# PrimeIntellect-ai/prime

Hardware: AMD Instinct MI355X
Metric: tokens_per_sec (higher is better)
Workload: dtype bf16; 1 GPU; model=intellect_10b, global_batch=8, seq_len=2048, parallelism=diloco1_h100_int8ring

## Files before the change

prime_amd/ops/_lib.py:

```python
from __future__ import annotations

import ctypes
from typing import Optional

import torch

from .build import LIB_PATH, build, needs_build

_LIB: Optional[ctypes.CDLL] = None
_TRIED = False

_SIGS = {
    "prime_rmsnorm_fwd": [ctypes.c_void_p] * 5 + [ctypes.c_int64] * 2 + [ctypes.c_double],
    "prime_rmsnorm_bwd": [ctypes.c_void_p] * 7 + [ctypes.c_int64] * 3 + [ctypes.c_double],
    "prime_add_rmsnorm_fwd": [ctypes.c_void_p] * 7 + [ctypes.c_int64] * 2 + [ctypes.c_double],
    "prime_add_rmsnorm_bwd": [ctypes.c_void_p] * 8 + [ctypes.c_int64] * 3 + [ctypes.c_double],
    "prime_rope": [ctypes.c_void_p] * 5 + [ctypes.c_int64] * 4 + [ctypes.c_int, ctypes.c_int64, ctypes.c_void_p],
    "prime_rope_strided": [ctypes.c_void_p] * 5 + [ctypes.c_int64] * 7,
    "prime_qkv_grad_pack": [ctypes.c_void_p] * 8 + [ctypes.c_int64] * 6,
    "prime_swiglu_bwd_t": [ctypes.c_void_p] * 5 + [ctypes.c_int64] * 2,
    "prime_swiglu_fwd": [ctypes.c_void_p] * 3 + [ctypes.c_int64] * 2,
    "prime_swiglu_bwd": [ctypes.c_void_p] * 4 + [ctypes.c_int64] * 2,
    "prime_adamw": [ctypes.c_void_p] * 7 + [ctypes.c_int64] + [ctypes.c_double] * 5 + [ctypes.c_int64],
    "prime_grad_sqnorm": [ctypes.c_void_p] * 3 + [ctypes.c_int64] * 2,
    "prime_grad_sqnorm_partials": [],
    "prime_pseudograd": [ctypes.c_void_p] * 4 + [ctypes.c_int64],
    "prime_quant_int8": [ctypes.c_void_p] * 4 + [ctypes.c_int64],
    "prime_dequant_int8": [ctypes.c_void_p] * 4 + [ctypes.c_int64] * 2,
    "prime_nesterov_outer": [ctypes.c_void_p] * 6 + [ctypes.c_int64] + [ctypes.c_double] * 2,
    "prime_cross_entropy": [ctypes.c_void_p] * 5 + [ctypes.c_int64] * 2 + [ctypes.c_double] + [ctypes.c_int64] * 2,
    "prime_flash_fwd": [ctypes.c_void_p] * 6 + [ctypes.c_int64] * 5 + [ctypes.c_double] + [ctypes.c_int64] * 7 + [ctypes.c_void_p],
    "prime_flash_bwd_dq": [ctypes.c_void_p] * 9 + [ctypes.c_int64] * 5 + [ctypes.c_double] + [ctypes.c_int64] * 10 + [ctypes.c_void_p],
    "prime_attn_delta_t": [ctypes.c_void_p] * 6 + [ctypes.c_int64] * 4,
    "prime_flash_bwd_dkv": [ctypes.c_void_p] * 12 + [ctypes.c_int64] * 6 + [ctypes.c_double] + [ctypes.c_int64] * 10 + [ctypes.c_void_p],
    "prime_flash_bwd_dkv_direct": [ctypes.c_int64] * 6,
    "prime_mfma_probe": [ctypes.c_void_p] * 4,
    "prime_mfma_probe32": [ctypes.c_void_p] * 4,
    "prime_transpose_bshd": [ctypes.c_void_p] * 3 + [ctypes.c_int64] * 7,
    "prime_attn_decode": [ctypes.c_void_p] * 5 + [ctypes.c_int64] * 6 + [ctypes.c_double, ctypes.c_void_p],
    "prime_attn_decode_ragged": [ctypes.c_void_p] * 7 + [ctypes.c_int64] * 6 + [ctypes.c_double],
    "prime_decode_ragged_chunk": [],
    "prime_decode_qkv_append": [ctypes.c_void_p] * 8 + [ctypes.c_int64] * 6,
    "prime_attn_decode_ragged_fp8": [ctypes.c_void_p] * 9 + [ctypes.c_int64] * 6 + [ctypes.c_double],
    "prime_decode_qkv_append_fp8": [ctypes.c_void_p] * 10 + [ctypes.c_int64] * 6,
    "prime_kv_store_fp8": [ctypes.c_void_p] * 7 + [ctypes.c_int64] * 6,
    "prime_gemm_nt": [ctypes.c_void_p] * 4 + [ctypes.c_int64] * 4,
    "prime_gemm_nt8": [ctypes.c_void_p] * 4 + [ctypes.c_int64] * 4,
    "prime_quant_fp8": [ctypes.c_void_p] * 6 + [ctypes.c_int64] * 2,
    "prime_rowwise_quant_fp8": [ctypes.c_void_p] * 4 + [ctypes.c_int64] * 3,
    "prime_transpose_fp8": [ctypes.c_void_p] * 3 + [ctypes.c_int64] * 7 + [ctypes.c_void_p] * 3 + [ctypes.c_int64],
}


def _load() -> ctypes.CDLL:
    import os

    override = os.environ.get("PRIME_AMD_LIB_PATH")
    path = override or str(LIB_PATH)
    if override is None and needs_build():
        build(verbose=True)
    lib = ctypes.CDLL(path)
    for name, argtypes in _SIGS.items():
        try:
            fn = getattr(lib, name)
        except AttributeError:
            continue
        fn.argtypes = argtypes
        fn.restype = ctypes.c_int
    return lib


def lib() -> ctypes.CDLL:
    global _LIB, _TRIED
    if _LIB is None:
        if _TRIED:
            raise RuntimeError("prime_amd HIP kernel library failed to load earlier")
        _TRIED = True
        try:
            _LIB = _load()
        except Exception as e:
            raise RuntimeError(
                "prime_amd requires its HIP kernel library on GPU machines; "
                f"build failed or .so missing at {LIB_PATH}: {e}"
            ) from e
    return _LIB


def have_lib() -> bool:
    try:
        lib()
        return True
    except RuntimeError:
        return False


def stream_of(t: torch.Tensor) -> ctypes.c_void_p:
    s = torch.cuda.current_stream(t.device).cuda_stream
    return ctypes.c_void_p(s)


def check(ret: int, what: str) -> None:
    if ret != 0:
        raise RuntimeError(f"HIP kernel {what} failed with hipError_t={ret}")


def ptr(t: Optional[torch.Tensor]) -> ctypes.c_void_p:
    if t is None:
        return ctypes.c_void_p(0)
    return ctypes.c_void_p(t.data_ptr())
```

prime_amd/ops/csrc/add_rmsnorm.hip:

```cpp
#include "common.h"

__global__ void add_rmsnorm_fwd_kernel(const bf16* __restrict__ x,
                                       const bf16* __restrict__ res,
                                       const bf16* __restrict__ w,
                                       bf16* __restrict__ s_out,
                                       bf16* __restrict__ y,
                                       float* __restrict__ rstd, int64_t R,
                                       int D, float eps) {
  __shared__ float scratch[16];
  const int tid = threadIdx.x;
  const int nthr = blockDim.x;
  const int dvec = D / 8;
  for (int64_t r = blockIdx.x; r < R; r += gridDim.x) {
    const bf16x8* xr = reinterpret_cast<const bf16x8*>(x + r * D);
    const bf16x8* rr = res ? reinterpret_cast<const bf16x8*>(res + r * D) : nullptr;
    bf16x8* sr = reinterpret_cast<bf16x8*>(s_out + r * D);
    float ss = 0.f;
    for (int i = tid; i < dvec; i += nthr) {
      bf16x8 v = xr[i], o;
#pragma unroll
      for (int j = 0; j < 8; ++j) {
        float f = bf2f(v.v[j]);
        if (rr) f += bf2f(rr[i].v[j]);
        o.v[j] = f2bf(f);
        ss += f * f;
      }
      sr[i] = o;
    }
    ss = block_reduce_sum(ss, scratch);
    const float rs = rsqrtf(ss / (float)D + eps);
    if (tid == 0) rstd[r] = rs;
    bf16x8* yr = reinterpret_cast<bf16x8*>(y + r * D);
    const bf16x8* wv = reinterpret_cast<const bf16x8*>(w);
    for (int i = tid; i < dvec; i += nthr) {
      bf16x8 v = sr[i], wj = wv[i], o;
#pragma unroll
      for (int j = 0; j < 8; ++j) o.v[j] = f2bf(bf2f(v.v[j]) * rs * bf2f(wj.v[j]));
      yr[i] = o;
    }
  }
}

__global__ void add_rmsnorm_bwd_kernel(const bf16* __restrict__ dy,
                                       const bf16* __restrict__ ds_res,
                                       const bf16* __restrict__ s,
                                       const bf16* __restrict__ w,
                                       const float* __restrict__ rstd,
                                       bf16* __restrict__ ds_out,
                                       float* __restrict__ dw_part, int64_t R,
                                       int D, float eps) {
  extern __shared__ float lds[];
  float* dw_loc = lds;
  float* scratch = lds + D;
  const int tid = threadIdx.x;
  const int nthr = blockDim.x;
  const int dvec = D / 8;
  for (int i = tid; i < D; i += nthr) dw_loc[i] = 0.f;
  __syncthreads();

  for (int64_t r = blockIdx.x; r < R; r += gridDim.x) {
    const bf16x8* dyr = reinterpret_cast<const bf16x8*>(dy + r * D);
    const bf16x8* srr = reinterpret_cast<const bf16x8*>(s + r * D);
    const bf16x8* dres = ds_res ? reinterpret_cast<const bf16x8*>(ds_res + r * D) : nullptr;
    const bf16x8* wv = reinterpret_cast<const bf16x8*>(w);
    const float rs = rstd[r];
    float dot = 0.f;
    for (int i = tid; i < dvec; i += nthr) {
      bf16x8 d = dyr[i], sv = srr[i], wj = wv[i];
#pragma unroll
      for (int j = 0; j < 8; ++j)
        dot += bf2f(d.v[j]) * bf2f(wj.v[j]) * bf2f(sv.v[j]) * rs;
    }
    dot = block_reduce_sum(dot, scratch);
    const float mean_dot = dot / (float)D;
    bf16x8* dso = reinterpret_cast<bf16x8*>(ds_out + r * D);
    for (int i = tid; i < dvec; i += nthr) {
      bf16x8 d = dyr[i], sv = srr[i], wj = wv[i], o;
#pragma unroll
      for (int j = 0; j < 8; ++j) {
        const float shat = bf2f(sv.v[j]) * rs;
        const float dyw = bf2f(d.v[j]) * bf2f(wj.v[j]);
        float g = rs * (dyw - shat * mean_dot);
        if (dres) g += bf2f(dres[i].v[j]);
        o.v[j] = f2bf(g);
        dw_loc[i * 8 + j] += bf2f(d.v[j]) * shat;
      }
      dso[i] = o;
    }
    __syncthreads();
  }
  for (int i = tid; i < D; i += nthr)
    dw_part[(int64_t)blockIdx.x * D + i] = dw_loc[i];
}

PRIME_API int prime_add_rmsnorm_fwd(hipStream_t stream, const void* x,
                                    const void* res, const void* w, void* s_out,
                                    void* y, void* rstd, int64_t R, int64_t D,
                                    double eps) {
  if (D % 8 != 0) return hipErrorInvalidValue;
  int grid = prime_grid(R, 1);
  hipLaunchKernelGGL(add_rmsnorm_fwd_kernel, dim3(grid), dim3(256), 0, stream,
                     (const bf16*)x, (const bf16*)res, (const bf16*)w,
                     (bf16*)s_out, (bf16*)y, (float*)rstd, R, (int)D,
                     (float)eps);
  return (int)hipGetLastError();
}

PRIME_API int prime_add_rmsnorm_bwd(hipStream_t stream, const void* dy,
                                    const void* ds_res, const void* s,
                                    const void* w, const void* rstd,
                                    void* ds_out, void* dw_part, int64_t R,
                                    int64_t D, int64_t dw_rows, double eps) {
  if (D % 8 != 0) return hipErrorInvalidValue;
  if (dw_rows < 1 || dw_rows > 1024) return hipErrorInvalidValue;
  int grid = (int)dw_rows;
  size_t lds = (size_t)(D + 16) * sizeof(float);
  if (lds > 160 * 1024 - 1024) return hipErrorInvalidValue;
  hipLaunchKernelGGL(add_rmsnorm_bwd_kernel, dim3(grid), dim3(256), lds,
                     stream, (const bf16*)dy, (const bf16*)ds_res,
                     (const bf16*)s, (const bf16*)w, (const float*)rstd,
                     (bf16*)ds_out, (float*)dw_part, R, (int)D, (float)eps);
  return (int)hipGetLastError();
}
```

prime_amd/ops/csrc/attention.hip:

```cpp
#include "common.h"
#include <stdlib.h>
#include <type_traits>

typedef __attribute__((ext_vector_type(8))) short short8;
typedef __attribute__((ext_vector_type(4))) float f32x4;
typedef __attribute__((address_space(3))) char lds_char;
typedef __attribute__((address_space(3))) void lds_void;
typedef __attribute__((address_space(1))) const void g_void;

__device__ __forceinline__ short8 ld8(const bf16* p) {
  return *reinterpret_cast<const short8*>(p);
}

__device__ __forceinline__ f32x4 mfma16(short8 a, short8 b, f32x4 c) {
  return __builtin_amdgcn_mfma_f32_16x16x32_bf16(a, b, c, 0, 0, 0);
}

__device__ __forceinline__ float grp16_max(float x) {
#pragma unroll
  for (int off = 1; off < 16; off <<= 1) x = fmaxf(x, __shfl_xor(x, off, 64));
  return x;
}
__device__ __forceinline__ float grp16_sum(float x) {
#pragma unroll
// ... 317 lines not shown
          o_acc[dt][r] *= bcast[(r & 3) + 8 * (r >> 2) + 4 * hi];
    }
    float psum = 0.f;
#pragma unroll
    for (int t = 0; t < 2; ++t)
#pragma unroll
      for (int r = 0; r < 16; ++r) {
        const float pv = (st[t][r] <= NEG_INF) ? 0.f : __expf(st[t][r] - m_run);
        st[t][r] = pv;
        psum += pv;
      }
    psum += __shfl_xor(psum, 32, 64);
    l_run = l_run * alpha + psum;

    short8 pa[2 * 2];
#pragma unroll
    for (int t = 0; t < 2; ++t) {
#pragma unroll
      for (int kst = 0; kst < 2; ++kst) {
        const int g0 = 4 * (2 * kst), g1 = 4 * (2 * kst + 1);
        unsigned x0 = cvt_pk_bf16(st[t][g0 + 0], st[t][g0 + 1]);
        unsigned x1 = cvt_pk_bf16(st[t][g0 + 2], st[t][g0 + 3]);
        unsigned y0 = cvt_pk_bf16(st[t][g1 + 0], st[t][g1 + 1]);
        unsigned y1 = cvt_pk_bf16(st[t][g1 + 2], st[t][g1 + 3]);
        permlane32_swap(x0, y0);
        permlane32_swap(x1, y1);
        short8 frag;
        reinterpret_cast<unsigned*>(&frag)[0] = x0;
        reinterpret_cast<unsigned*>(&frag)[1] = x1;
        reinterpret_cast<unsigned*>(&frag)[2] = y0;
        reinterpret_cast<unsigned*>(&frag)[3] = y1;
        pa[t * 2 + kst] = frag;
      }
    }
#pragma unroll
    for (int dt = 0; dt < DT32; ++dt)
#pragma unroll
      for (int ks = 0; ks < 4; ++ks)
        o_acc[dt] = mfma32(pa[ks],
                           ld8_swz<64>(vt_lds[idx], dt * 32 + lo, ks * 32 + hi * 16),
                           o_acc[dt]);
  }
  if (hi == 0) bcast[lo] = (l_run > 0.f) ? 1.f / l_run : 0.f;
  wave_lds_fence();
#pragma unroll
  for (int r = 0; r < 16; ++r) {
    const int qr = (r & 3) + 8 * (r >> 2) + 4 * hi;
    const float inv = bcast[qr];
    bf16* orow = O + (((int64_t)(b * S + q0w + qr)) * H + h) * D;
#pragma unroll
    for (int dt = 0; dt < DT32; ++dt)
      orow[dt * 32 + lo] = f2bf(o_acc[dt][r] * inv);
  }
  if (hi == 0)
    lse[((int64_t)(b * S + q0w + lo)) * H + h] = m_run + __logf(fmaxf(l_run, 1e-30f));
}

__global__ void attn_delta_kernel(const bf16* __restrict__ dO,
                                  const bf16* __restrict__ O,
                                  float* __restrict__ delta, int64_t rows,
                                  int D, const float* __restrict__ lse,
                                  float* __restrict__ rowc_t, int S, int H) {
  const int64_t row0 = (int64_t)blockIdx.x * (blockDim.x >> 6) + (threadIdx.x >> 6);
  const int lane = threadIdx.x & 63;
  for (int64_t r = row0; r < rows; r += (int64_t)gridDim.x * (blockDim.x >> 6)) {
    float acc = 0.f;
    for (int i = lane * 2; i < D; i += 128) {
      acc += bf2f(dO[r * D + i]) * bf2f(O[r * D + i]);
      acc += bf2f(dO[r * D + i + 1]) * bf2f(O[r * D + i + 1]);
    }
    acc = wave_reduce_sum(acc);
    if (lane == 0) {
      delta[r] = acc;
      if (rowc_t) {
        const int64_t bs = r / H;
        const int h = (int)(r - bs * H);
        const int64_t bb = bs / S;
        const int s = (int)(bs - bb * S);
        const int64_t t = (bb * H + h) * S + s;
        rowc_t[t] = lse[r];
        rowc_t[rows + t] = acc;
      }
    }
  }
}

template <int D, bool DOC = false>
__global__ __launch_bounds__(512, 2) void flash_bwd_dq_v5_kernel(
    const bf16* __restrict__ Q, const bf16* __restrict__ K,
    const bf16* __restrict__ V, const bf16* __restrict__ Kt,
    const bf16* __restrict__ dO, const float* __restrict__ lse,
    const float* __restrict__ delta, bf16* __restrict__ dQ, int B, int H,
    int Hkv, int S, float scale, int causal,
    int64_t sqb, int64_t sqs, int64_t sqh,
    int64_t skb, int64_t sks, int64_t skh,
    int64_t svb, int64_t svs, int64_t svh,
    const int* __restrict__ doc) {
  constexpr int DSL = D / 16;
  constexpr int DT32 = D / 32;
  const int n_qt = S / 256;
  const int nwg = gridDim.x;
  int vb = blockIdx.x;
  if ((nwg & 7) == 0) vb = (blockIdx.x & 7) * (nwg >> 3) + (blockIdx.x >> 3);
  const int bh = vb / n_qt;
  const int qt = n_qt - 1 - (vb - bh * n_qt);
  const int b = bh / H, h = bh - b * H;
  const int hkv = h / (H / Hkv);
  const int wid = threadIdx.x >> 6;
  const int lane = threadIdx.x & 63;
  const int lo = lane & 31, hi = lane >> 5;
  const int q0w = qt * 256 + wid * 32;

  const bf16* Qb = Q + b * sqb + h * sqh;
  const bf16* Kb = K + b * skb + hkv * skh;
  const bf16* Vb = V + b * svb + hkv * svh;
  const bf16* Ktb = Kt + ((int64_t)(b * Hkv + hkv) * D) * S;
  const bf16* dOb = dO + ((int64_t)b * S * H + h) * D;
  const float* lse_b = lse + (int64_t)b * S * H + h;
  const float* dl_b = delta + (int64_t)b * S * H + h;

  __shared__ bf16 k_lds[2][64 * D];
  __shared__ bf16 v_lds[2][64 * D];
  __shared__ bf16 kt_lds[2][D * 64];

  short8 qf[DSL], dof[DSL];
#pragma unroll
  for (int ds = 0; ds < DSL; ++ds) {
    const bf16* src = Qb + (int64_t)(q0w + lo) * sqs + ds * 16 + hi * 8;
    short8 raw = ld8(src);
    short8 sc;
#pragma unroll
    for (int j = 0; j < 8; ++j) {
      bf16 v = reinterpret_cast<const bf16*>(&raw)[j];
      reinterpret_cast<bf16*>(&sc)[j] = f2bf(bf2f(v) * scale);
    }
    qf[ds] = sc;
    dof[ds] = ld8(dOb + (int64_t)(q0w + lo) * H * D + ds * 16 + hi * 8);
  }
  const float lse_q = lse_b[(int64_t)(q0w + lo) * H];
  const float dl_q = dl_b[(int64_t)(q0w + lo) * H];

  f32x16 dq_acc[DT32];
#pragma unroll
  for (int dt = 0; dt < DT32; ++dt)
#pragma unroll
    for (int r = 0; r < 16; ++r) dq_acc[dt][r] = 0.f;

  const int kv_end = causal ? (qt * 256 + 256) : S;
  const int my_kv_end = causal ? (q0w + 32) : S;
  int kv_begin = 0, my_kv_begin = 0, my_ds = 0;
  if (DOC) {
    const int* doc_b = doc + (int64_t)b * S;
    kv_begin = doc_clamp(doc_b[qt * 256], qt * 256) & ~63;
    my_kv_begin = doc_clamp(doc_b[q0w], q0w) & ~63;
    my_ds = doc_b[q0w + lo];
  }
  stage_tile<64, D, 512>(Kb + (int64_t)kv_begin * sks, sks, k_lds[0], threadIdx.x);
  stage_tile<64, D, 512>(Vb + (int64_t)kv_begin * svs, svs, v_lds[0], threadIdx.x);
  stage_tile<D, 64, 512>(Ktb + kv_begin, S, kt_lds[0], threadIdx.x);
  int idx = 0;
  for (int kv = kv_begin; kv < kv_end; kv += 64, idx ^= 1) {
    __syncthreads();
    if (kv + 64 < kv_end) {
      stage_tile<64, D, 512>(Kb + (int64_t)(kv + 64) * sks, sks,
                             k_lds[idx ^ 1], threadIdx.x);
      stage_tile<64, D, 512>(Vb + (int64_t)(kv + 64) * svs, svs,
// ... 341 lines not shown
  }
  }
}

__global__ void dkv_reduce_kernel(const float* __restrict__ wsK,
                                  const float* __restrict__ wsV,
                                  bf16* __restrict__ dK, bf16* __restrict__ dV,
                                  int B, int Hkv, int S, int D, int splits) {
  const int64_t n = (int64_t)B * Hkv * S * D;
  for (int64_t i = (int64_t)blockIdx.x * blockDim.x + threadIdx.x; i < n;
       i += (int64_t)gridDim.x * blockDim.x) {
    float k = 0.f, v = 0.f;
    for (int sp = 0; sp < splits; ++sp) {
      k += wsK[(int64_t)sp * n + i];
      v += wsV[(int64_t)sp * n + i];
    }
    const int d = (int)(i % D);
    int64_t r = i / D;
    const int sq = (int)(r % S);
    r /= S;
    const int hk = (int)(r % Hkv);
    const int bb = (int)(r / Hkv);
    const int64_t o = (((int64_t)(bb * S + sq)) * Hkv + hk) * D + d;
    dK[o] = f2bf(k);
    dV[o] = f2bf(v);
  }
}

template <typename To, typename From>
static To kernel_arg(From v) {
  static_assert(std::is_pointer<To>::value == std::is_pointer<From>::value,
                "pointer / scalar mismatch in a kernel argument list");
  return (To)v;
}

template <typename... P, typename... A>
static int attn_launch(void (*kernel)(P...), int64_t grid, int block,
                       hipStream_t stream, A... args) {
  hipLaunchKernelGGL(kernel, dim3((int)grid), dim3(block), 0, stream,
                     kernel_arg<P>(args)...);
  return (int)hipGetLastError();
}

#define BY_D_DOC(LAUNCH)                                          \
  (D == 128 ? (doc ? LAUNCH(128, true) : LAUNCH(128, false))      \
            : (doc ? LAUNCH(64, true) : LAUNCH(64, false)))

static bool attn_use_v5(int64_t S) {
  static const char* v5env = getenv("PRIME_ATTN_V5");
  return (S % 256 == 0) && !(v5env && v5env[0] == '0');
}

PRIME_API int prime_flash_fwd(hipStream_t stream, const void* Q, const void* K,
                              const void* Vt, void* O, void* lse, int64_t B,
                              int64_t H, int64_t Hkv, int64_t S, int64_t D,
                              double scale, int64_t causal,
                              int64_t sqb, int64_t sqs, int64_t sqh,
                              int64_t skb, int64_t sks, int64_t skh,
                              const void* doc_start) {
  if (S % 64 != 0 || (D != 64 && D != 128)) return hipErrorInvalidValue;
  const bool doc = doc_start != nullptr;
  if (doc && !causal) return hipErrorInvalidValue;
  const bool v5 = attn_use_v5(S);
#define FWD(DD, DOCV)                                                        \
  attn_launch(v5 ? flash_fwd_v5_kernel<DD, DOCV>                             \
                 : flash_fwd_kernel<DD, 4, DOCV>,                            \
              B * H * (S / (v5 ? 256 : 64)), v5 ? 512 : 256, stream, Q, K,   \
              Vt, O, lse, B, H, Hkv, S, scale, causal, sqb, sqs, sqh, skb,   \
              sks, skh, doc_start)
  return BY_D_DOC(FWD);
#undef FWD
}

PRIME_API int prime_attn_delta_t(hipStream_t stream, const void* dO,
                                 const void* O, const void* lse, void* delta,
                                 void* rowc_t, int64_t B, int64_t S, int64_t H,
                                 int64_t D) {
  if (!lse || !rowc_t) return hipErrorInvalidValue;
  const int64_t rows = B * S * H;
  int grid = prime_grid(rows * 64, 256);
  hipLaunchKernelGGL(attn_delta_kernel, dim3(grid), dim3(256), 0, stream,
                     (const bf16*)dO, (const bf16*)O, (float*)delta, rows,
                     (int)D, (const float*)lse, (float*)rowc_t, (int)S, (int)H);
  return (int)hipGetLastError();
}

PRIME_API int prime_flash_bwd_dq(hipStream_t stream, const void* Q,
                                 const void* K, const void* V, const void* Kt,
                                 const void* dO, const void* lse,
                                 const void* delta, void* dQ, int64_t B,
                                 int64_t H, int64_t Hkv, int64_t S, int64_t D,
                                 double scale, int64_t causal,
                                 int64_t sqb, int64_t sqs, int64_t sqh,
                                 int64_t skb, int64_t sks, int64_t skh,
                                 int64_t svb, int64_t svs, int64_t svh,
                                 const void* doc_start) {
  if (S % 64 != 0 || (D != 64 && D != 128)) return hipErrorInvalidValue;
  const bool doc = doc_start != nullptr;
  if (doc && !causal) return hipErrorInvalidValue;
  const bool v5 = attn_use_v5(S);
#define DQ(DD, DOCV)                                                         \
  attn_launch(v5 ? flash_bwd_dq_v5_kernel<DD, DOCV>                          \
                 : flash_bwd_dq_kernel<DD, DOCV>,                            \
              B * H * (S / (v5 ? 256 : 64)), v5 ? 512 : 256, stream, Q, K,   \
              V, Kt, dO, lse, delta, dQ, B, H, Hkv, S, scale, causal, sqb,   \
              sqs, sqh, skb, sks, skh, svb, svs, svh, doc_start)
  return BY_D_DOC(DQ);
#undef DQ
}

static int64_t dkv_tile_rows(int64_t S) { return (S % 128 == 0) ? 128 : 64; }

PRIME_API int prime_flash_bwd_dkv_direct(int64_t B, int64_t Hkv, int64_t S,
                                         int64_t D, int64_t causal,
                                         int64_t has_doc) {
  const char* env = getenv("PRIME_ATTN_DKV_DIRECT");
  if (env && env[0] == '1') return 1;
  if (env && env[0] == '0') return 0;
  static int n_cu = 0;
  if (n_cu == 0) {
    int dev = 0, n = 0;
    if (hipGetDevice(&dev) != hipSuccess ||
        hipDeviceGetAttribute(&n, hipDeviceAttributeMultiprocessorCount, dev) != hipSuccess ||
        n <= 0)
      n = 256;
    n_cu = n;
  }
  const int64_t n_kt = S / dkv_tile_rows(S);
  const int64_t blocks = B * Hkv * (causal ? (n_kt + 1) / 2 : n_kt);
  return blocks >= n_cu ? 1 : 0;
}

PRIME_API int prime_flash_bwd_dkv(hipStream_t stream, const void* Q,
                                  const void* Qt, const void* K, const void* V,
                                  const void* dO, const void* dOt,
                                  const void* rowc, void* dK,
                                  void* dV, void* wsK, void* wsV,
                                  int64_t splits, int64_t B, int64_t H,
                                  int64_t Hkv, int64_t S, int64_t D,
                                  double scale, int64_t causal,
                                  int64_t sqb, int64_t sqs, int64_t sqh,
                                  int64_t skb, int64_t sks, int64_t skh,
                                  int64_t svb, int64_t svs, int64_t svh,
                                  const void* doc_end) {
  if (S % 64 != 0 || (D != 64 && D != 128)) return hipErrorInvalidValue;
  const bool doc = doc_end != nullptr;
  if (doc && !causal) return hipErrorInvalidValue;
  const bool direct =
      prime_flash_bwd_dkv_direct(B, Hkv, S, D, causal, doc) != 0;
  if (splits < 1) return hipErrorInvalidValue;
  if ((!direct || splits > 1) && (!wsK || !wsV)) return hipErrorInvalidValue;
  if (!rowc) return hipErrorInvalidValue;
  const bool nw8 = dkv_tile_rows(S) == 128;
  const int64_t n_kt = S / dkv_tile_rows(S);
  const int64_t per_bh = (direct && causal) ? (n_kt + 1) / 2 : n_kt;
#define DKV(DD, DOCV)                                                        \
  attn_launch(nw8 ? flash_bwd_dkv_kernel<DD, 8, 2, DOCV>                     \
                  : flash_bwd_dkv_kernel<DD, 4, 1, DOCV>,                    \
              B * Hkv * per_bh * (direct ? 1 : splits), nw8 ? 512 : 256,     \
              stream, Q, Qt, K, V, dO, dOt, rowc, wsK, wsV, dK, dV, B, H,    \
              Hkv, S, scale, causal, splits, direct, sqb, sqs, sqh, skb,     \
              sks, skh, svb, svs, svh, doc_end)
  int err = BY_D_DOC(DKV);
#undef DKV
  if (err || direct) return err;
  int rgrid = prime_grid(B * Hkv * S * D, 256);
// ... 6 lines not shown
```

prime_amd/ops/functional.py:

```python
from __future__ import annotations

import os
from typing import NamedTuple

import torch

from . import reference as ref
from ._lib import check, lib, ptr, stream_of

_DW_ROWS = 1024


def _is_hip(t: torch.Tensor) -> bool:
    return t.is_cuda


class _RMSNorm(torch.autograd.Function):
    @staticmethod
    def forward(ctx, x: torch.Tensor, w: torch.Tensor, eps: float):
        if not _is_hip(x):
            ctx.save_for_backward(x, w)
            ctx.eps = eps
            return ref.rmsnorm(x, w, eps)
        x = x.contiguous()
# ... 238 lines not shown
    new_doc = torch.zeros(B, S, dtype=torch.bool, device=tokens.device)
    new_doc[:, 1:] = tokens[:, :-1] == eos_id
    return torch.where(new_doc, idx, torch.zeros_like(idx)).cummax(dim=1).values


def _doc_ends(doc_start: torch.Tensor) -> torch.Tensor:
    B, S = doc_start.shape
    idx = torch.arange(S, device=doc_start.device, dtype=torch.int32).expand(B, S)
    cand = torch.where(doc_start == idx, idx, torch.full_like(idx, S))
    nxt = cand.flip(1).cummin(dim=1).values.flip(1)
    return torch.cat([nxt[:, 1:], torch.full_like(idx[:, :1], S)], dim=1).contiguous()


_DOC_END_CACHE: list = [None, None, None]


def _doc_ends_cached(doc_start: torch.Tensor) -> torch.Tensor:
    import weakref

    ref_, ver, val = _DOC_END_CACHE
    if ref_ is not None and ref_() is doc_start and ver == doc_start._version:
        return val
    val = _doc_ends(doc_start)
    _DOC_END_CACHE[:] = [weakref.ref(doc_start), doc_start._version, val]
    return val


def _check_doc_start(doc_start, q, causal: bool) -> None:
    B, S = q.shape[0], q.shape[1]
    if not causal:
        raise ValueError("flash_attention: doc_start requires causal=True")
    if not isinstance(doc_start, torch.Tensor) or doc_start.dtype != torch.int32:
        raise TypeError(
            "flash_attention: doc_start must be an int32 tensor "
            f"(got {getattr(doc_start, 'dtype', type(doc_start))})")
    if tuple(doc_start.shape) != (B, S):
        raise ValueError(
            f"flash_attention: doc_start must have shape [B, S] = [{B}, {S}] "
            f"(got {list(doc_start.shape)})")
    if doc_start.device != q.device:
        raise ValueError(
            f"flash_attention: doc_start is on {doc_start.device}, q on {q.device}")


class _FlashAttention(torch.autograd.Function):

    @staticmethod
    def forward(ctx, q, k, v, causal: bool, scale: float, doc_start=None):
        B, S, H, D = q.shape
        _check_flash_shape(S, D)
        Hkv = k.shape[2]
        if not (_bshd_ok(q) and _bshd_ok(k) and _bshd_ok(v)):
            q, k, v = q.contiguous(), k.contiguous(), v.contiguous()
        if doc_start is not None:
            doc_start = doc_start.contiguous()
        vt = transpose_bshd(v)
        o = torch.empty(B, S, H, D, device=q.device, dtype=q.dtype)
        lse = torch.empty(B, S, H, device=q.device, dtype=torch.float32)
        check(
            lib().prime_flash_fwd(
                stream_of(q), ptr(q), ptr(k), ptr(vt), ptr(o), ptr(lse),
                B, H, Hkv, S, D, scale, int(causal),
                q.stride(0), q.stride(1), q.stride(2),
                k.stride(0), k.stride(1), k.stride(2), ptr(doc_start),
            ),
            "flash_fwd",
        )
        ctx.save_for_backward(q, k, v, o, lse)
        ctx.meta = (causal, scale)
        ctx.doc_start = doc_start
        return o

    @staticmethod
    def backward(ctx, do):
        q, k, v, o, lse = ctx.saved_tensors
        causal, scale = ctx.meta
        doc_start = ctx.doc_start
        doc_end = _doc_ends_cached(doc_start) if doc_start is not None else None
        B, S, H, D = q.shape
        Hkv = k.shape[2]
        do = do.contiguous()
        delta = torch.empty(B * S * H, device=q.device, dtype=torch.float32)
        rowc = torch.empty(2, B, H, S, device=q.device, dtype=torch.float32)
        check(
            lib().prime_attn_delta_t(stream_of(q), ptr(do), ptr(o), ptr(lse), ptr(delta),
                                     ptr(rowc), B, S, H, D),
            "attn_delta",
        )
        kt = transpose_bshd(k)
        dq = torch.empty(B, S, H, D, device=q.device, dtype=q.dtype)
        check(
            lib().prime_flash_bwd_dq(
                stream_of(q), ptr(q), ptr(k), ptr(v), ptr(kt), ptr(do),
                ptr(lse), ptr(delta), ptr(dq), B, H, Hkv, S, D, scale,
                int(causal),
                q.stride(0), q.stride(1), q.stride(2),
                k.stride(0), k.stride(1), k.stride(2),
                v.stride(0), v.stride(1), v.stride(2), ptr(doc_start),
            ),
            "flash_bwd_dq",
        )
        qt = transpose_bshd(q)
        dot = transpose_bshd(do)
        dk = torch.empty(B, S, Hkv, D, device=q.device, dtype=q.dtype)
        dv = torch.empty(B, S, Hkv, D, device=q.device, dtype=q.dtype)
        direct = bool(lib().prime_flash_bwd_dkv_direct(
            B, Hkv, S, D, int(causal), int(doc_end is not None)))
        env = os.environ.get("PRIME_AMD_DKV_SPLITS")
        if env:
            splits = max(1, min(int(env), S // 64))
        else:
            splits = max(1, min(8, S // 1024, S // 64))
        ws_slices = (0 if splits == 1 else 1) if direct else splits
        ws = torch.empty(2, ws_slices, B, Hkv, S, D, device=q.device,
                         dtype=torch.float32) if ws_slices else None
        check(
            lib().prime_flash_bwd_dkv(
                stream_of(q), ptr(q), ptr(qt), ptr(k), ptr(v), ptr(do),
                ptr(dot), ptr(rowc), ptr(dk), ptr(dv),
                ptr(None if ws is None else ws[0]), ptr(None if ws is None else ws[1]), splits,
                B, H, Hkv, S, D, scale, int(causal),
                q.stride(0), q.stride(1), q.stride(2),
                k.stride(0), k.stride(1), k.stride(2),
                v.stride(0), v.stride(1), v.stride(2), ptr(doc_end),
            ),
            "flash_bwd_dkv",
        )
        return dq, dk, dv, None, None, None


def flash_attention(q, k, v, causal: bool = True, doc_start=None) -> torch.Tensor:
    if doc_start is not None:
        _check_doc_start(doc_start, q, causal)
    if not _is_hip(q):
        return ref.attention(q, k, v, causal, doc_start=doc_start)
    if doc_start is None:
        return _FlashAttention.apply(q, k, v, causal, q.shape[-1] ** -0.5)
    return _FlashAttention.apply(q, k, v, causal, q.shape[-1] ** -0.5, doc_start)


class _CrossEntropy(torch.autograd.Function):
    @staticmethod
    def forward(ctx, logits, targets, ignore_index: int, need_grad: bool):
        R, V = logits.shape
        logits = logits.contiguous()
        t32 = targets.to(torch.int32).contiguous()
        loss = torch.empty(R, device=logits.device, dtype=torch.float32)
        dlogits = torch.empty_like(logits) if need_grad else logits
        check(
            lib().prime_cross_entropy(
                stream_of(logits), ptr(logits), ptr(t32), ptr(loss), ptr(dlogits),
                R, V, 1.0, ignore_index, 1 if need_grad else 0,
            ),
            "cross_entropy",
        )
        n_valid = (targets != ignore_index).sum().clamp(min=1)
        if need_grad:
            ctx.save_for_backward(dlogits, n_valid)
        else:
            ctx.save_for_backward(torch.empty(0, device=logits.device,
                                              dtype=logits.dtype), n_valid)
        return loss.sum() / n_valid.float()

    @staticmethod
    def backward(ctx, grad_out):
        dlogits, n_valid = ctx.saved_tensors
        g = dlogits * (grad_out.float() / n_valid.float()).to(dlogits.dtype)
        return g, None, None, None


def cross_entropy(logits, targets, ignore_index: int = -100) -> torch.Tensor:
    if not _is_hip(logits):
        return ref.cross_entropy(logits, targets, ignore_index)
    need_grad = torch.is_grad_enabled() and logits.requires_grad
    return _CrossEntropy.apply(logits, targets, ignore_index, need_grad)


_WT_EPOCH = 0
_WT_CACHE: dict = {}
_LINEAR_TUNED = False


def set_linear_tuned(on: bool) -> None:
    global _LINEAR_TUNED
    _LINEAR_TUNED = bool(on)
    _WT_CACHE.clear()
# ... 796 lines not shown
```

Before: 17150 tokens/s.

## Add register-resident add_rmsnorm kernels and fuse attention delta with dO transpose

Adds templated add_rmsnorm forward and backward kernels that keep a whole row in registers, reuse the weight across rows, and prefetch the next row while the current one is reduced. Backward dw partials now accumulate in registers instead of LDS. The change also adds an attention-backward kernel that computes delta and rowc and writes the transposed dO in the same pass, which removes a separate transpose launch and a second read of dO. The risks are register pressure from large per-thread row arrays, a changed floating-point operation order, and extra LDS tile use in the delta kernel.

```diff
diff --git a/prime_amd/ops/_lib.py b/prime_amd/ops/_lib.py
--- a/prime_amd/ops/_lib.py
+++ b/prime_amd/ops/_lib.py
@@ -15,6 +15,8 @@
     "prime_rmsnorm_bwd": [ctypes.c_void_p] * 7 + [ctypes.c_int64] * 3 + [ctypes.c_double],
     "prime_add_rmsnorm_fwd": [ctypes.c_void_p] * 7 + [ctypes.c_int64] * 2 + [ctypes.c_double],
     "prime_add_rmsnorm_bwd": [ctypes.c_void_p] * 8 + [ctypes.c_int64] * 3 + [ctypes.c_double],
+    "prime_add_rmsnorm_fwd_generic": [ctypes.c_void_p] * 7 + [ctypes.c_int64] * 2 + [ctypes.c_double],
+    "prime_add_rmsnorm_bwd_generic": [ctypes.c_void_p] * 8 + [ctypes.c_int64] * 3 + [ctypes.c_double],
     "prime_rope": [ctypes.c_void_p] * 5 + [ctypes.c_int64] * 4 + [ctypes.c_int, ctypes.c_int64, ctypes.c_void_p],
     "prime_rope_strided": [ctypes.c_void_p] * 5 + [ctypes.c_int64] * 7,
     "prime_qkv_grad_pack": [ctypes.c_void_p] * 8 + [ctypes.c_int64] * 6,
@@ -32,6 +34,7 @@
     "prime_flash_fwd": [ctypes.c_void_p] * 6 + [ctypes.c_int64] * 5 + [ctypes.c_double] + [ctypes.c_int64] * 7 + [ctypes.c_void_p],
     "prime_flash_bwd_dq": [ctypes.c_void_p] * 9 + [ctypes.c_int64] * 5 + [ctypes.c_double] + [ctypes.c_int64] * 10 + [ctypes.c_void_p],
     "prime_attn_delta_t": [ctypes.c_void_p] * 6 + [ctypes.c_int64] * 4,
+    "prime_attn_delta_dot": [ctypes.c_void_p] * 7 + [ctypes.c_int64] * 4,
     "prime_flash_bwd_dkv": [ctypes.c_void_p] * 12 + [ctypes.c_int64] * 6 + [ctypes.c_double] + [ctypes.c_int64] * 10 + [ctypes.c_void_p],
     "prime_flash_bwd_dkv_direct": [ctypes.c_int64] * 6,
     "prime_mfma_probe": [ctypes.c_void_p] * 4,
diff --git a/prime_amd/ops/csrc/add_rmsnorm.hip b/prime_amd/ops/csrc/add_rmsnorm.hip
--- a/prime_amd/ops/csrc/add_rmsnorm.hip
+++ b/prime_amd/ops/csrc/add_rmsnorm.hip
@@ -1,4 +1,34 @@
 #include "common.h"
+
+__device__ __forceinline__ float nrm_add(float x, float r) {
+#pragma clang fp contract(off)
+  return x + r;
+}
+__device__ __forceinline__ float nrm_sq_acc(float ss, float f) {
+  return __builtin_fmaf(f, f, ss);
+}
+__device__ __forceinline__ float nrm_y(float s, float rs, float w) {
+#pragma clang fp contract(off)
+  return s * rs * w;
+}
+__device__ __forceinline__ float nrm_dot_acc(float dot, float d, float w,
+                                             float s, float rs) {
+#pragma clang fp contract(off)
+  return dot + d * w * s * rs;
+}
+__device__ __forceinline__ float nrm_shat(float s, float rs) {
+#pragma clang fp contract(off)
+  return s * rs;
+}
+__device__ __forceinline__ float nrm_g(float d, float w, float shat,
+                                       float mean_dot, float rs) {
+#pragma clang fp contract(off)
+  const float t = shat * mean_dot;
+  return rs * __builtin_fmaf(d, w, -t);
+}
+__device__ __forceinline__ float nrm_dw_acc(float dw, float d, float shat) {
+  return __builtin_fmaf(d, shat, dw);
+}
 
 __global__ void add_rmsnorm_fwd_kernel(const bf16* __restrict__ x,
                                        const bf16* __restrict__ res,
@@ -21,9 +51,9 @@
 #pragma unroll
       for (int j = 0; j < 8; ++j) {
         float f = bf2f(v.v[j]);
-        if (rr) f += bf2f(rr[i].v[j]);
+        if (rr) f = nrm_add(f, bf2f(rr[i].v[j]));
         o.v[j] = f2bf(f);
-        ss += f * f;
+        ss = nrm_sq_acc(ss, f);
       }
       sr[i] = o;
     }
@@ -35,7 +65,7 @@
     for (int i = tid; i < dvec; i += nthr) {
       bf16x8 v = sr[i], wj = wv[i], o;
 #pragma unroll
-      for (int j = 0; j < 8; ++j) o.v[j] = f2bf(bf2f(v.v[j]) * rs * bf2f(wj.v[j]));
+      for (int j = 0; j < 8; ++j) o.v[j] = f2bf(nrm_y(bf2f(v.v[j]), rs, bf2f(wj.v[j])));
       yr[i] = o;
     }
   }
@@ -69,7 +99,7 @@
       bf16x8 d = dyr[i], sv = srr[i], wj = wv[i];
 #pragma unroll
       for (int j = 0; j < 8; ++j)
-        dot += bf2f(d.v[j]) * bf2f(wj.v[j]) * bf2f(sv.v[j]) * rs;
+        dot = nrm_dot_acc(dot, bf2f(d.v[j]), bf2f(wj.v[j]), bf2f(sv.v[j]), rs);
     }
     dot = block_reduce_sum(dot, scratch);
     const float mean_dot = dot / (float)D;
@@ -78,12 +108,11 @@
       bf16x8 d = dyr[i], sv = srr[i], wj = wv[i], o;
 #pragma unroll
       for (int j = 0; j < 8; ++j) {
-        const float shat = bf2f(sv.v[j]) * rs;
-        const float dyw = bf2f(d.v[j]) * bf2f(wj.v[j]);
-        float g = rs * (dyw - shat * mean_dot);
-        if (dres) g += bf2f(dres[i].v[j]);
+        const float shat = nrm_shat(bf2f(sv.v[j]), rs);
+        float g = nrm_g(bf2f(d.v[j]), bf2f(wj.v[j]), shat, mean_dot, rs);
+        if (dres) g = nrm_add(g, bf2f(dres[i].v[j]));
         o.v[j] = f2bf(g);
-        dw_loc[i * 8 + j] += bf2f(d.v[j]) * shat;
+        dw_loc[i * 8 + j] = nrm_dw_acc(dw_loc[i * 8 + j], bf2f(d.v[j]), shat);
       }
       dso[i] = o;
     }
@@ -93,10 +122,199 @@
     dw_part[(int64_t)blockIdx.x * D + i] = dw_loc[i];
 }
 
-PRIME_API int prime_add_rmsnorm_fwd(hipStream_t stream, const void* x,
-                                    const void* res, const void* w, void* s_out,
-                                    void* y, void* rstd, int64_t R, int64_t D,
-                                    double eps) {
+template <int NV>
+__device__ __forceinline__ bool nrm_owns(int k, int tid, int dvec) {
+  return k < NV - 1 || tid + k * 256 < dvec;
+}
+
+template <int NV>
+__device__ __forceinline__ void nrm_offsets(int tid, int dvec, unsigned (&off)[NV]) {
+#pragma unroll
+  for (int k = 0; k < NV; ++k) {
+    const int i = tid + k * 256;
+    off[k] = 16u * (unsigned)(k < NV - 1 ? i : min(i, dvec - 1));
+  }
+}
+
+template <int NV>
+__device__ __forceinline__ void nrm_load_row(const bf16* __restrict__ row,
+                                             const unsigned (&off)[NV],
+                                             bf16x8 (&v)[NV]) {
+  const char* p = reinterpret_cast<const char*>(row);
+#pragma unroll
+  for (int k = 0; k < NV; ++k) v[k] = *reinterpret_cast<const bf16x8*>(p + off[k]);
+}
+
+__device__ __forceinline__ void nrm_store(bf16* __restrict__ row, unsigned off,
+                                          const bf16x8& v) {
+  *reinterpret_cast<bf16x8*>(reinterpret_cast<char*>(row) + off) = v;
+}
+
+__device__ __forceinline__ void nrm_pin(bf16x8& v) {
+  typedef unsigned u32x4 __attribute__((ext_vector_type(4)));
+  u32x4 u = __builtin_bit_cast(u32x4, v);
+  asm volatile("" : "+v"(u));
+  v = __builtin_bit_cast(bf16x8, u);
+}
+
+#define NRM_FWD_WAVES(NV) ((NV) <= 2 ? 8 : 4)
+#define NRM_BWD_WAVES(NV) ((NV) <= 2 ? 4 : 2)
+
+template <int NV, bool HAS_RES>
+__global__ __launch_bounds__(256, NRM_FWD_WAVES(NV)) void add_rmsnorm_fwd_rows_kernel(
+    const bf16* __restrict__ x, const bf16* __restrict__ res,
+    const bf16* __restrict__ w, bf16* __restrict__ s_out, bf16* __restrict__ y,
+    float* __restrict__ rstd, int64_t R, int D, float eps) {
+  __shared__ float scratch[16];
+  const int tid = threadIdx.x;
+  const int dvec = D / 8;
+  unsigned off[NV];
+  nrm_offsets<NV>(tid, dvec, off);
+  bf16x8 wj[NV], xv[NV], rv[NV];
+  nrm_load_row<NV>(w, off, wj);
+  int64_t r = blockIdx.x;
+  if (r < R) {
+    nrm_load_row<NV>(x + r * D, off, xv);
+    if (HAS_RES) nrm_load_row<NV>(res + r * D, off, rv);
+#pragma unroll
+    for (int k = 0; k < NV; ++k) {
+      nrm_pin(xv[k]);
+      if (HAS_RES) nrm_pin(rv[k]);
+      nrm_pin(wj[k]);
+    }
+  }
+  for (; r < R; r += gridDim.x) {
+    bf16x8 sv[NV];
+    float ss = 0.f;
+#pragma unroll
+    for (int k = 0; k < NV; ++k) nrm_pin(wj[k]);
+#pragma unroll
+    for (int k = 0; k < NV; ++k) {
+      const bool own = nrm_owns<NV>(k, tid, dvec);
+#pragma unroll
+      for (int j = 0; j < 8; ++j) {
+        float f = bf2f(xv[k].v[j]);
+        if (HAS_RES) f = nrm_add(f, bf2f(rv[k].v[j]));
+        sv[k].v[j] = f2bf(f);
+        const float acc = nrm_sq_acc(ss, f);
+        ss = own ? acc : ss;
+      }
+    }
+    const int64_t rn = r + gridDim.x;
+    if (rn < R) {
+      nrm_load_row<NV>(x + rn * D, off, xv);
+      if (HAS_RES) nrm_load_row<NV>(res + rn * D, off, rv);
+    }
+#pragma unroll
+    for (int k = 0; k < NV; ++k)
+      if (nrm_owns<NV>(k, tid, dvec)) nrm_store(s_out + r * D, off[k], sv[k]);
+    ss = block_reduce_sum(ss, scratch);
+    const float rs = rsqrtf(ss / (float)D + eps);
+    if (tid == 0) rstd[r] = rs;
+#pragma unroll
+    for (int k = 0; k < NV; ++k) {
+      bf16x8 o;
+#pragma unroll
+      for (int j = 0; j < 8; ++j)
+        o.v[j] = f2bf(nrm_y(bf2f(sv[k].v[j]), rs, bf2f(wj[k].v[j])));
+      if (nrm_owns<NV>(k, tid, dvec)) nrm_store(y + r * D, off[k], o);
+    }
+  }
+}
+
+template <int NV, bool HAS_DRES>
+__global__ __launch_bounds__(256, NRM_BWD_WAVES(NV)) void add_rmsnorm_bwd_rows_kernel(
+    const bf16* __restrict__ dy, const bf16* __restrict__ ds_res,
+    const bf16* __restrict__ s, const bf16* __restrict__ w,
+    const float* __restrict__ rstd, bf16* __restrict__ ds_out,
+    float* __restrict__ dw_part, int64_t R, int D, float eps) {
+  __shared__ float scratch[16];
+  const int tid = threadIdx.x;
+  const int dvec = D / 8;
+  bf16x8 wj[NV], dv[NV], sv[NV], rv[NV];
+  float dw[NV][8];
+#pragma unroll
+  for (int k = 0; k < NV; ++k)
+#pragma unroll
+    for (int j = 0; j < 8; ++j) dw[k][j] = 0.f;
+  unsigned off[NV];
+  nrm_offsets<NV>(tid, dvec, off);
+  nrm_load_row<NV>(w, off, wj);
+  int64_t r = blockIdx.x;
+  float rs = 0.f;
+  if (r < R) {
+    nrm_load_row<NV>(dy + r * D, off, dv);
+    nrm_load_row<NV>(s + r * D, off, sv);
+    if (HAS_DRES) nrm_load_row<NV>(ds_res + r * D, off, rv);
+    rs = rstd[r];
+#pragma unroll
+    for (int k = 0; k < NV; ++k) {
+      nrm_pin(dv[k]);
+      nrm_pin(sv[k]);
+      if (HAS_DRES) nrm_pin(rv[k]);
+      nrm_pin(wj[k]);
+    }
+  }
+  for (; r < R; r += gridDim.x) {
+    bf16x8 dk[NV], sk[NV], rk[NV];
+    const float rsr = rs;
+    float dot = 0.f;
+#pragma unroll
+    for (int k = 0; k < NV; ++k) nrm_pin(wj[k]);
+#pragma unroll
+    for (int k = 0; k < NV; ++k) {
+      const bool own = nrm_owns<NV>(k, tid, dvec);
+      dk[k] = dv[k];
+      sk[k] = sv[k];
+      if (HAS_DRES) rk[k] = rv[k];
+#pragma unroll
+      for (int j = 0; j < 8; ++j) {
+        const float acc = nrm_dot_acc(dot, bf2f(dk[k].v[j]), bf2f(wj[k].v[j]),
+                                      bf2f(sk[k].v[j]), rsr);
+        dot = own ? acc : dot;
+      }
+    }
+    const int64_t rn = r + gridDim.x;
+    if (rn < R) {
+      nrm_load_row<NV>(dy + rn * D, off, dv);
+      nrm_load_row<NV>(s + rn * D, off, sv);
+      if (HAS_DRES) nrm_load_row<NV>(ds_res + rn * D, off, rv);
+      rs = rstd[rn];
+    }
+    dot = block_reduce_sum(dot, scratch);
+    const float mean_dot = dot / (float)D;
+#pragma unroll
+    for (int k = 0; k < NV; ++k) {
+      bf16x8 o;
+#pragma unroll
+      for (int j = 0; j < 8; ++j) {
+        const float d = bf2f(dk[k].v[j]);
+        const float shat = nrm_shat(bf2f(sk[k].v[j]), rsr);
+        float g = nrm_g(d, bf2f(wj[k].v[j]), shat, mean_dot, rsr);
+        if (HAS_DRES) g = nrm_add(g, bf2f(rk[k].v[j]));
+        o.v[j] = f2bf(g);
+        dw[k][j] = nrm_dw_acc(dw[k][j], d, shat);
+      }
+      if (nrm_owns<NV>(k, tid, dvec)) nrm_store(ds_out + r * D, off[k], o);
+    }
+  }
+  float* dwo = dw_part + (int64_t)blockIdx.x * D;
+#pragma unroll
+  for (int k = 0; k < NV; ++k) {
+    if (!nrm_owns<NV>(k, tid, dvec)) continue;
+    f32x4v lo, hi;
+#pragma unroll
+    for (int j = 0; j < 4; ++j) { lo.v[j] = dw[k][j]; hi.v[j] = dw[k][4 + j]; }
+    f32x4v* p = reinterpret_cast<f32x4v*>(dwo + (int64_t)(tid + k * 256) * 8);
+    p[0] = lo;
+    p[1] = hi;
+  }
+}
+
+static int add_rmsnorm_fwd_generic(hipStream_t stream, const void* x,
+                                   const void* res, const void* w, void* s_out,
+                                   void* y, void* rstd, int64_t R, int64_t D,
+                                   double eps) {
   if (D % 8 != 0) return hipErrorInvalidValue;
   int grid = prime_grid(R, 1);
   hipLaunchKernelGGL(add_rmsnorm_fwd_kernel, dim3(grid), dim3(256), 0, stream,
@@ -106,11 +324,11 @@
   return (int)hipGetLastError();
 }
 
-PRIME_API int prime_add_rmsnorm_bwd(hipStream_t stream, const void* dy,
-                                    const void* ds_res, const void* s,
-                                    const void* w, const void* rstd,
-                                    void* ds_out, void* dw_part, int64_t R,
-                                    int64_t D, int64_t dw_rows, double eps) {
+static int add_rmsnorm_bwd_generic(hipStream_t stream, const void* dy,
+                                   const void* ds_res, const void* s,
+                                   const void* w, const void* rstd,
+                                   void* ds_out, void* dw_part, int64_t R,
+                                   int64_t D, int64_t dw_rows, double eps) {
   if (D % 8 != 0) return hipErrorInvalidValue;
   if (dw_rows < 1 || dw_rows > 1024) return hipErrorInvalidValue;
   int grid = (int)dw_rows;
@@ -122,3 +340,79 @@
                      (bf16*)ds_out, (float*)dw_part, R, (int)D, (float)eps);
   return (int)hipGetLastError();
 }
+
+static int nrm_rows_nv(int64_t D) {
+  if (D < 8 || D % 8 != 0 || D > 8192) return 0;
+  return (int)((D / 8 + 255) / 256);
+}
+
+PRIME_API int prime_add_rmsnorm_fwd_generic(hipStream_t stream, const void* x,
+                                            const void* res, const void* w,
+                                            void* s_out, void* y, void* rstd,
+                                            int64_t R, int64_t D, double eps) {
+  return add_rmsnorm_fwd_generic(stream, x, res, w, s_out, y, rstd, R, D, eps);
+}
+
+PRIME_API int prime_add_rmsnorm_bwd_generic(hipStream_t stream, const void* dy,
+                                            const void* ds_res, const void* s,
+                                            const void* w, const void* rstd,
+                                            void* ds_out, void* dw_part,
+                                            int64_t R, int64_t D,
+                                            int64_t dw_rows, double eps) {
+  return add_rmsnorm_bwd_generic(stream, dy, ds_res, s, w, rstd, ds_out,
+                                 dw_part, R, D, dw_rows, eps);
+}
+
+PRIME_API int prime_add_rmsnorm_fwd(hipStream_t stream, const void* x,
+                                    const void* res, const void* w, void* s_out,
+                                    void* y, void* rstd, int64_t R, int64_t D,
+                                    double eps) {
+  const int nv = nrm_rows_nv(D);
+  if (nv == 0)
+    return add_rmsnorm_fwd_generic(stream, x, res, w, s_out, y, rstd, R, D, eps);
+  const int grid = prime_grid(R, 1);
+#define FWD_ROWS(NV, HAS)                                                     \
+  hipLaunchKernelGGL((add_rmsnorm_fwd_rows_kernel<NV, HAS>), dim3(grid),      \
+                     dim3(256), 0, stream, (const bf16*)x, (const bf16*)res,  \
+                     (const bf16*)w, (bf16*)s_out, (bf16*)y, (float*)rstd, R, \
+                     (int)D, (float)eps)
+#define FWD_ROWS_NV(NV) do { if (res) FWD_ROWS(NV, true); else FWD_ROWS(NV, false); } while (0)
+  switch (nv) {
+    case 1: FWD_ROWS_NV(1); break;
+    case 2: FWD_ROWS_NV(2); break;
+    case 3: FWD_ROWS_NV(3); break;
+    default: FWD_ROWS_NV(4); break;
+  }
+#undef FWD_ROWS_NV
+#undef FWD_ROWS
+  return (int)hipGetLastError();
+}
+
+PRIME_API int prime_add_rmsnorm_bwd(hipStream_t stream, const void* dy,
+                                    const void* ds_res, const void* s,
+                                    const void* w, const void* rstd,
+                                    void* ds_out, void* dw_part, int64_t R,
+                                    int64_t D, int64_t dw_rows, double eps) {
+  const int nv = nrm_rows_nv(D);
+  if (nv == 0)
+    return add_rmsnorm_bwd_generic(stream, dy, ds_res, s, w, rstd, ds_out,
+                                   dw_part, R, D, dw_rows, eps);
+  if (dw_rows < 1 || dw_rows > 1024) return hipErrorInvalidValue;
+  const int grid = (int)dw_rows;
+#define BWD_ROWS(NV, HAS)                                                     \
+  hipLaunchKernelGGL((add_rmsnorm_bwd_rows_kernel<NV, HAS>), dim3(grid),      \
+                     dim3(256), 0, stream, (const bf16*)dy,                   \
+                     (const bf16*)ds_res, (const bf16*)s, (const bf16*)w,     \
+                     (const float*)rstd, (bf16*)ds_out, (float*)dw_part, R,   \
+                     (int)D, (float)eps)
+#define BWD_ROWS_NV(NV) do { if (ds_res) BWD_ROWS(NV, true); else BWD_ROWS(NV, false); } while (0)
+  switch (nv) {
+    case 1: BWD_ROWS_NV(1); break;
+    case 2: BWD_ROWS_NV(2); break;
+    case 3: BWD_ROWS_NV(3); break;
+    default: BWD_ROWS_NV(4); break;
+  }
+#undef BWD_ROWS_NV
+#undef BWD_ROWS
+  return (int)hipGetLastError();
+}
diff --git a/prime_amd/ops/csrc/attention.hip b/prime_amd/ops/csrc/attention.hip
--- a/prime_amd/ops/csrc/attention.hip
+++ b/prime_amd/ops/csrc/attention.hip
@@ -423,6 +423,85 @@
         rowc_t[rows + t] = acc;
       }
     }
+  }
+}
+
+template <int D>
+__global__ __launch_bounds__(256) void attn_delta_dot_kernel(
+    const bf16* __restrict__ dO, const bf16* __restrict__ O,
+    const float* __restrict__ lse, float* __restrict__ delta,
+    float* __restrict__ rowc_t, bf16* __restrict__ dOt, int S, int H,
+    int64_t rows) {
+  constexpr int LPR = D / 8;
+  constexpr int RPP = 256 / LPR;
+  constexpr int NP = 64 / RPP;
+  constexpr int TPD = D + 8;
+  __shared__ __attribute__((aligned(16))) bf16 tile[64][TPD];
+  __shared__ float sdelta[64];
+  int idx = blockIdx.x;
+  const int h = idx % H; idx /= H;
+  const int n_st = S / 64;
+  const int st = idx % n_st;
+  const int b = idx / n_st;
+  const int t = threadIdx.x;
+  const int m = t % LPR, rr = t / LPR;
+  const int64_t tok0 = (int64_t)b * S + st * 64;
+  const int64_t tcol = ((int64_t)b * H + h) * S + st * 64;
+
+  short8 vdo[NP], vo[NP];
+#pragma unroll
+  for (int p = 0; p < NP; ++p) {
+    const int64_t off = ((tok0 + p * RPP + rr) * H + h) * D + m * 8;
+    vdo[p] = *reinterpret_cast<const short8*>(dO + off);
+    vo[p] = *reinterpret_cast<const short8*>(O + off);
+  }
+  float lv = 0.f;
+  if (t >= 64 && t < 128) lv = lse[(tok0 + (t - 64)) * H + h];
+
+#pragma unroll
+  for (int p = 0; p < NP; ++p) {
+    const int row = p * RPP + rr;
+    *reinterpret_cast<short8*>(&tile[row][m * 8]) = vdo[p];
+    const bf16* a = reinterpret_cast<const bf16*>(&vdo[p]);
+    const bf16* c = reinterpret_cast<const bf16*>(&vo[p]);
+    float q[4];
+#pragma unroll
+    for (int i = 0; i < 4; ++i) {
+      float acc = 0.f;
+      acc += bf2f(a[2 * i]) * bf2f(c[2 * i]);
+      acc += bf2f(a[2 * i + 1]) * bf2f(c[2 * i + 1]);
+      q[i] = acc;
+    }
+#pragma unroll
+    for (int i = 0; i < 4; ++i) {
+      if (D == 64) q[i] = q[i] + 0.f;
+      else q[i] += __shfl_down(q[i], 8, 64);
+    }
+#pragma unroll
+    for (int off = 4; off > 0; off >>= 1)
+#pragma unroll
+      for (int i = 0; i < 4; ++i) q[i] += __shfl_down(q[i], off, 64);
+    if (m == 0) sdelta[row] = (q[0] + q[2]) + (q[1] + q[3]);
+  }
+  __syncthreads();
+  if (t < 64) {
+    const float d = sdelta[t];
+    delta[(tok0 + t) * H + h] = d;
+    rowc_t[rows + tcol + t] = d;
+  } else if (t < 128) {
+    rowc_t[tcol + (t - 64)] = lv;
+  }
+  bf16* dbase = dOt + ((int64_t)b * H + h) * D * S + st * 64;
+#pragma unroll
+  for (int i = 0; i < D / 32; ++i) {
+    const int u = i * 256 + t;
+    const int d = u >> 3, s8 = (u & 7) * 8;
+    short8 v;
+#pragma unroll
+    for (int j = 0; j < 8; ++j)
+      reinterpret_cast<short*>(&v)[j] =
+          reinterpret_cast<const short*>(&tile[s8 + j][d])[0];
+    *reinterpret_cast<short8*>(dbase + (int64_t)d * S + s8) = v;
   }
 }
 
@@ -930,6 +1009,29 @@
   hipLaunchKernelGGL(attn_delta_kernel, dim3(grid), dim3(256), 0, stream,
                      (const bf16*)dO, (const bf16*)O, (float*)delta, rows,
                      (int)D, (const float*)lse, (float*)rowc_t, (int)S, (int)H);
+  return (int)hipGetLastError();
+}
+
+PRIME_API int prime_attn_delta_dot(hipStream_t stream, const void* dO,
+                                   const void* O, const void* lse, void* delta,
+                                   void* rowc_t, void* dOt, int64_t B,
+                                   int64_t S, int64_t H, int64_t D) {
+  if (!dO || !O || !lse || !delta || !rowc_t || !dOt) return hipErrorInvalidValue;
+  if (S % 64 != 0 || (D != 64 && D != 128)) return hipErrorInvalidValue;
+  const int64_t rows = B * S * H;
+  const int64_t grid = B * H * (S / 64);
+  if (grid > 0x7fffffff) return hipErrorInvalidValue;
+  if (grid == 0) return (int)hipSuccess;
+  if (D == 64)
+    hipLaunchKernelGGL(attn_delta_dot_kernel<64>, dim3((int)grid), dim3(256), 0,
+                       stream, (const bf16*)dO, (const bf16*)O,
+                       (const float*)lse, (float*)delta, (float*)rowc_t,
+                       (bf16*)dOt, (int)S, (int)H, rows);
+  else
+    hipLaunchKernelGGL(attn_delta_dot_kernel<128>, dim3((int)grid), dim3(256),
+                       0, stream, (const bf16*)dO, (const bf16*)O,
+                       (const float*)lse, (float*)delta, (float*)rowc_t,
+                       (bf16*)dOt, (int)S, (int)H, rows);
   return (int)hipGetLastError();
 }
 
diff --git a/prime_amd/ops/functional.py b/prime_amd/ops/functional.py
--- a/prime_amd/ops/functional.py
+++ b/prime_amd/ops/functional.py
@@ -344,10 +344,11 @@
         do = do.contiguous()
         delta = torch.empty(B * S * H, device=q.device, dtype=torch.float32)
         rowc = torch.empty(2, B, H, S, device=q.device, dtype=torch.float32)
+        dot = torch.empty(B, H, D, S, device=q.device, dtype=q.dtype)
         check(
-            lib().prime_attn_delta_t(stream_of(q), ptr(do), ptr(o), ptr(lse), ptr(delta),
-                                     ptr(rowc), B, S, H, D),
-            "attn_delta",
+            lib().prime_attn_delta_dot(stream_of(q), ptr(do), ptr(o), ptr(lse), ptr(delta),
+                                       ptr(rowc), ptr(dot), B, S, H, D),
+            "attn_delta_dot",
         )
         kt = transpose_bshd(k)
         dq = torch.empty(B, S, H, D, device=q.device, dtype=q.dtype)
@@ -363,7 +364,6 @@
             "flash_bwd_dq",
         )
         qt = transpose_bshd(q)
-        dot = transpose_bshd(do)
         dk = torch.empty(B, S, Hkv, D, device=q.device, dtype=q.dtype)
         dv = torch.empty(B, S, Hkv, D, device=q.device, dtype=q.dtype)
         direct = bool(lib().prime_flash_bwd_dkv_direct(
```

After: 17380 tokens/s (median of 6 runs). 1.3% higher.
